# voidstar69/softray

Hardware: AMD Instinct MI355X
Metric: Mrays/s (primary rays) at 4096x4096, shading + 100-sample soft shadows, own BVH, frame read back to the host (higher is better)
Workload: dtype f64; 1 GPU; 1000000 random triangles (System.Random seed 12345, extent 0.05, unit cube) + BVH, 4096x4096, spp 1, shading + 100 shadow samples/hit, pose yaw135/pitch-22/depth 1.5; trace_mode=bvh, parallelism=one GPU

## Files before the change

softray_amd/csrc/sr_api.cpp:

```cpp
#include "../../include/softray.h"

#include <hip/hip_runtime.h>

#include <algorithm>
#include <climits>
#include <cmath>
#include <cstdio>
#include <cstdlib>
#include <cstring>
#include <memory>
#include <string>
#include <vector>

#include "sr_device.h"
#include "sr_host.h"
#include "sr_rccl.h"

namespace {

thread_local std::string g_err;

int fail(int code, const std::string& msg) {
    g_err = msg;
    return code;
// ... 8 lines not shown
        if (e__ != hipSuccess) return hip_fail(e__, #call);  \
    } while (0)

int rccl_fail(const sr::RcclApi* api, int rc, const char* what) {
    g_err = std::string(what) + ": " + (api && api->GetErrorString ? api->GetErrorString(rc) : "RCCL error") + " (" + std::to_string(rc) + ")";
    return SR_ERR_HIP;
}
#define SR_RCCL(api, call)                                        \
    do {                                                          \
        int r__ = (call);                                         \
        if (r__ != 0) return rccl_fail(api, r__, #call);          \
    } while (0)

struct DBuf {
    void*  p = nullptr;
    size_t cap = 0;
    hipError_t reserve(size_t bytes) {
        if (bytes <= cap && p) return hipSuccess;
        if (p) { hipError_t e = hipFree(p); p = nullptr; cap = 0; if (e != hipSuccess) return e; }
        size_t want = std::max<size_t>(bytes, 256);
        hipError_t e = hipMalloc(&p, want);
        if (e == hipSuccess) cap = want;
        return e;
    }
    template <class T> hipError_t upload(const std::vector<T>& v) {
        hipError_t e = reserve(v.size() * sizeof(T));
        if (e != hipSuccess || v.empty()) return e;
        return hipMemcpy(p, v.data(), v.size() * sizeof(T), hipMemcpyHostToDevice);
    }
    void release() { if (p) (void)hipFree(p); p = nullptr; cap = 0; }
};

}

struct sr_scene {
    int device = -1;
    std::vector<sr_scene*> parts;
    std::vector<double>   v9;
    std::vector<uint32_t> argb;
    double bmin[3] = {0, 0, 0}, bmax[3] = {0, 0, 0};
    double vmin[3] = {0, 0, 0}, vmax[3] = {0, 0, 0};
    bool have_model = false;
    size_t ntris = 0;
    const sr_scene* host_src = nullptr;
    bool host_model_stale = false;
    std::vector<sr::Rec128> tri_recs;
    std::vector<sr::Rec128> extra_recs;
    sr::RootBox root{};
    sr::RefTree ref;
    sr::Bvh     bvh;
    bool        bvh_on_device = false;
    size_t      bvh_num_nodes = 0;
    DBuf d_tris, d_extra, d_rnodes, d_rboxes, d_rleaf, d_bnodes, d_btris, d_bslab, d_v9, d_bcam;
    DBuf d_bounds;
    std::vector<int> b4_level_first;
    DBuf d_bdepth, d_tbox;
    bool bdepth_valid = false;
    double cam_origin[3] = {0, 0, 0};
    bool   cam_valid = false;
    DBuf   d_blight;
    bool   blight_valid = false;
    double blight_pos[3] = {0, 0, 0}, blight_radius = 0;
    DBuf   d_binter;
    bool   interior_valid = false;
    DBuf d_b4, d_b4cam, d_b4light;
    size_t b4_num = 0;
    int    b4_depth = 0;
    bool   b4cam_valid = false, b4light_valid = false;
    int    b4cam_known = 0, b4light_known = 0;
    DBuf   d_rng_cam, d_rng_light;
    bool   part_valid = false, part_cam = false, part_light = false;
    double part_origin[3] = {0, 0, 0}, part_lightpos[3] = {0, 0, 0}, part_radius = 0;
    double b4_light[3] = {0, 0, 0};
    double b4_light_radius = 0;
    uint32_t dbg_frame[3] = {0, 0, 0};
    hipEvent_t pre_ready = nullptr, pre_used = nullptr;
    bool pre_ready_set = false, pre_used_set = false;
    DBuf d_shadow_cache, d_static_claim, d_static_hits;
    DBuf d_ao_cache, d_ao_claim;
    DBuf d_aop_table, d_aop_rows, d_aop_state;
    DBuf d_pp_state;
    bool aop_rows_ready = false;
    std::unique_ptr<sr::NetRandom> aop_host_random;
    uint64_t aop_host_drawn = 0;
    bool ao_cache_empty = true;
    std::vector<uint8_t> ao_cache_host;
    std::vector<uint8_t> shadow_cache_host;
    int32_t ao_table_seed = 0;
    int  ao_table_rc = SR_OK;
    DBuf d_lf_cache, d_lf_claim, d_lf_points;
    int32_t lf_res = 64;
    bool lf_shadows = false;
    bool lf_interp = false;
    int32_t lf_points_res = 0;
    bool lf_cache_empty = true;
    std::vector<uint32_t> lf_cache_host;
    bool lf_tris = false;
    DBuf d_lft_cache, d_lft_claim, d_rhandle;
    bool lft_cache_empty = true;
    std::vector<uint32_t> lft_cache_host;
    DBuf d_pt_table;
    int32_t pt_table_seed = 0;
// ... 629 lines not shown
    const bool shadows_on_bvh = (fc.flags & SR_F_SHADOWS) && f->trace_mode == SR_MODE_REF_TREE && !(f->flags & SR_F_LITERAL_SECONDARY) && s->bvh.built && !static_shadows &&
                                (fc.flags & SR_F_POINT_LIGHT) && fc.shadow_samples <= kMaxShaftSamples && f->max_bounces == 0 &&
                                !(f->flags & (SR_F_SINGLE_KERNEL | SR_F_PER_LANE_SHADOWS)) && s->dbg[SR_DBG_LITERAL_SHADOWS] <= 0;
    if (shadows_on_bvh && (rc = sync_geometry(s, SR_MODE_BVH))) return rc;
    const bool bvh_walks = f->trace_mode == SR_MODE_BVH || shadows_on_bvh;
    const bool wide = bvh_walks && s->b4_num > 0 && s->dbg[SR_DBG_BVH2_PACKETS] <= 0;
    bool rewrote = false;
    const bool lf = (f->flags & SR_F_LIGHT_FIELD) != 0;
    const bool pkt_primary = f->trace_mode == SR_MODE_BVH && s->dbg[SR_DBG_PER_LANE_PRIMARY] <= 0 && !((f->flags & SR_F_FOCAL_BLUR) && f->sub_pixel_res > 1) && !lf && !pts;
    const bool want_cam = wide && pkt_primary, want_light = wide && (fc.flags & SR_F_SHADOWS) && (fc.flags & SR_F_POINT_LIGHT);
    if ((want_cam || want_light) && s->dbg[SR_DBG_KERNEL_SWITCH] != 71) {
        const auto same3 = [](const double* a, const double* b) { return a[0] == b[0] && a[1] == b[1] && a[2] == b[2]; };
        const bool cam_ok = !want_cam || (s->part_cam && same3(s->part_origin, fc.start_world));
        const bool light_ok = !want_light || (s->part_light && same3(s->part_lightpos, fc.light_pos_model) && s->part_radius == fc.light_radius);
        if (!s->part_valid || !cam_ok || !light_ok) {
            SR_HIP(s->d_rng_cam.reserve(s->b4_num * 4 * 8));
            SR_HIP(s->d_rng_light.reserve(s->b4_num * 4 * 8));
            rewrote = true;
            s->part_valid = false;
            s->cam_valid = false; s->b4cam_valid = false; s->b4light_valid = false;
            s->blight_valid = false;
            s->interior_valid = false;
            SR_HIP(sr::launch_facing_partition((const sr::Bvh4Node*)s->d_b4.p, (int)s->b4_num, (sr::Rec128*)s->d_btris.p, (sr::TriSlab*)s->d_bslab.p,
                                               fc.start_world, want_cam, fc.light_pos_model, fc.light_radius, want_light, s->d_rng_cam.p, s->d_rng_light.p, stream));
            s->part_cam = want_cam; s->part_light = want_light;
            for (int i = 0; i < 3; ++i) { s->part_origin[i] = fc.start_world[i]; s->part_lightpos[i] = fc.light_pos_model[i]; }
            s->part_radius = fc.light_radius;
            s->part_valid = true;
        }
    } else if (s->part_valid && s->dbg[SR_DBG_KERNEL_SWITCH] == 71) {
        s->part_valid = false; s->b4cam_valid = false; s->b4light_valid = false;
        s->blight_valid = false;
    }
    if (bvh_walks && (fc.flags & SR_F_SHADOWS) && (fc.flags & SR_F_POINT_LIGHT) && s->d_bslab.p && !s->interior_valid) {
        SR_HIP(s->d_binter.reserve(s->ntris));
        rewrote = true;
        SR_HIP(sr::launch_interior_flags(dev_scene(s), (int)s->ntris, (uint8_t*)s->d_binter.p, stream));
        s->interior_valid = true;
    }
    if (pkt_primary) {
        const size_t nt = s->ntris;
        const bool same_origin = s->cam_origin[0] == fc.start_world[0] && s->cam_origin[1] == fc.start_world[1] && s->cam_origin[2] == fc.start_world[2];
        if (!s->cam_valid || !same_origin) {
            SR_HIP(s->d_bcam.reserve(nt * sizeof(sr::CamCone)));
            rewrote = true;
            s->cam_valid = false;
            s->b4cam_valid = false;
            SR_HIP(sr::launch_cam_cones(dev_scene(s), (int)nt, fc.start_world, (sr::CamCone*)s->d_bcam.p, stream));
            for (int i = 0; i < 3; ++i) s->cam_origin[i] = fc.start_world[i];
            s->cam_valid = true;
        }
        if (wide && !s->b4cam_valid) {
            rewrote = true;
            int known, swap;
            point_outside_axes(s->root, fc.start_world, 0.0, known, swap);
            if (known != 7 || s->dbg[SR_DBG_KERNEL_SWITCH] == 61) known = swap = 0;
            SR_HIP(sr::launch_order_nodes((const sr::Bvh4Node*)s->d_b4.p, (sr::Bvh4Node*)s->d_b4cam.p, (int)s->b4_num, s->root, fc.start_world, false, swap,
                                          (s->part_valid && s->part_cam) ? s->d_rng_cam.p : nullptr, stream));
            s->b4cam_known = known;
            s->b4cam_valid = true;
        }
        if (wide) s->dbg_frame[0] |= (uint32_t)s->b4cam_known << 4;
    }
    if (wide && (fc.flags & SR_F_SHADOWS) && (fc.flags & SR_F_POINT_LIGHT)) {
        const bool same_light = s->b4_light[0] == fc.light_pos_model[0] && s->b4_light[1] == fc.light_pos_model[1] && s->b4_light[2] == fc.light_pos_model[2] &&
                                s->b4_light_radius == fc.light_radius;
        if (!s->b4light_valid || !same_light) {
            rewrote = true;
            s->b4light_valid = false;
            int known, beyond;
            point_outside_axes(s->root, fc.light_pos_model, fc.light_radius, known, beyond);
            if (s->dbg[SR_DBG_KERNEL_SWITCH] == 62) known = 0;
            SR_HIP(sr::launch_order_nodes((const sr::Bvh4Node*)s->d_b4.p, (sr::Bvh4Node*)s->d_b4light.p, (int)s->b4_num, s->root, fc.light_pos_model, true, known & ~beyond,
                                          (s->part_valid && s->part_light) ? s->d_rng_light.p : nullptr, stream));
            s->b4light_known = known;
            for (int i = 0; i < 3; ++i) s->b4_light[i] = fc.light_pos_model[i];
            s->b4_light_radius = fc.light_radius;
            s->b4light_valid = true;
        }
        s->dbg_frame[0] |= (uint32_t)s->b4light_known;
    }
    const bool shadows = (fc.flags & SR_F_SHADOWS) != 0;
    const bool shaft = shadows && bvh_walks && (fc.flags & SR_F_POINT_LIGHT) && !(f->flags & SR_F_PER_LANE_SHADOWS) &&
                       (fc.shadow_samples <= 128 || (fc.shadow_samples <= kMaxShaftSamples && !static_shadows));
    if (shaft && wide && s->b4light_valid && dev_scene(s).b4light && !(s->dbg[SR_DBG_PER_LANE_SHAFT] > 0 && (s->dbg[SR_DBG_PER_LANE_SHAFT] & 1)) &&
        s->dbg[SR_DBG_KERNEL_SWITCH] != 96) {
        const bool same_ball = s->blight_pos[0] == fc.light_pos_model[0] && s->blight_pos[1] == fc.light_pos_model[1] && s->blight_pos[2] == fc.light_pos_model[2] &&
                               s->blight_radius == fc.light_radius;
        if (!s->blight_valid || !same_ball) {
            s->blight_valid = false;
            if (s->d_blight.reserve(s->ntris * sizeof(sr::LightCone)) == hipSuccess) {
                rewrote = true;
                SR_HIP(sr::launch_light_cones(dev_scene(s), (int)s->ntris, fc.light_pos_model, fc.light_radius, (sr::LightCone*)s->d_blight.p, stream));
                for (int i = 0; i < 3; ++i) s->blight_pos[i] = fc.light_pos_model[i];
                s->blight_radius = fc.light_radius;
                s->blight_valid = true;
            } else {
                (void)hipGetLastError();
            }
        }
    } else if (s->dbg[SR_DBG_KERNEL_SWITCH] == 96) {
        s->blight_valid = false;
    }
    if (rewrote) {
        if (!s->pre_ready) SR_HIP(hipEventCreateWithFlags(&s->pre_ready, hipEventDisableTiming));
        SR_HIP(hipEventRecord(s->pre_ready, stream));
        s->pre_ready_set = true;
// ... 2603 lines not shown
```

softray_amd/csrc/sr_device.h:

```cpp
#pragma once
#include <hip/hip_runtime.h>
#include <stdint.h>

#include <vector>

#include "sr_types.h"

namespace sr {

struct DevScene {
    const Rec128*  tris;
    int32_t        ntris;
    const Rec128*  extra;
    int32_t        nextra;
    const RefNode* rnodes;
    const LeafBox* rboxes;
    const int32_t* rleaf;
    int32_t        rdepth;
    const BvhNode* bnodes;
    const Rec128*  btris;
    const TriSlab* bslab;
    const CamCone* bcam;
    const LightCone* blight;
    const double*  v9;
    int32_t        bdepth;
    int32_t        bnode_bits;
    const Bvh4Node* b4;
    const Bvh4Node* b4cam;
    const Bvh4Node* b4light;
    int32_t        b4depth;
    int32_t        b4cam_known, b4light_known;
    RootBox        root;
    uint8_t*       shadow_cache;
    const uint8_t* binter;
};

constexpr int kShaftRounds = 2;
enum KernelId { K_RENDER = 0, K_TRACE = 1, K_PRIMARY = 2, K_SHADOW = 3, K_RESOLVE = 4, K_SHAFT = 5, K_FALLBACK = 6, K_SHAFT2 = 7, K_SHADOW2 = 8, K_POST = 9, K_ANTI_ALIAS = 10, K_BOUNCE = 11, K_PATHTRACE = 12, K_PT_COUNT = 13, K_PT_EXCHANGE = 14, K_VOXEL_WALK = 15, K_VOXELISE = 16, K_AO = 17, K_AO_PROBE = 18, K_LF_LOOKUP = 19, K_LF_FILL = 20, K_LF_APPLY = 21, K_LF_BAKE = 22, K_TRI_RECORDS = 23, K_TRI_BOUNDS = 24, K_REFIT_LEAVES = 25, K_REFIT_NODES = 26, K_PTS_INGEST = 27, K_PTS_SORT = 28, K_LFI_LOOKUP = 29, K_LFI_APPLY = 30, K_LFT_FILL = 31, K_LFT_HIT = 32, K_LFT_TRACE = 33, K_LFT_BAKE = 34, K_HITS = 35, K_DRAWS = 36, K_AOP_PROBE = 37, K_PP_TRACE = 38, K_SSP_CLAIM = 39, K_SSP_APPLY = 40, K_COUNT = 41 };
const char* kernel_name(int id);

struct RenderLaunch {
    DevScene    sc;
    FrameConst  fc;
    int32_t     mode;
    const double* offsets;
    const int32_t* row_map;
    uint32_t*   pixels;
    unsigned long long* stats;
    hipStream_t stream;
};

hipError_t launch_render(const RenderLaunch& L);

struct HitsOut {
    double*   starts;
    double*   dirs;
    uint8_t*  hit;
    double*   ray_frac;
    double*   pos;
    double*   normal;
    uint32_t* color;
    int32_t*  tri;
};

struct PipelineLaunch {
    DevScene    sc;
    FrameConst  fc;
    int32_t     mode;
    const double*  offsets;
    const int32_t* row_map;
    uint32_t*   pixels;
// ... 165 lines not shown
    const double* pos;
    const double* nrm;
    const uint32_t* color;
    uint32_t*   out;
    uint32_t*   incoming;
    double*     dirs;
    uint64_t    first_sample;
    void*       rays;
    int32_t*    table;
    const NetState* windows;
    const uint32_t* stride_rows;
    int32_t*    base_window;
    uint32_t*   pass_units;
    hipError_t (*host_table)(void* user, uint64_t first_point, uint32_t count, int32_t* d_table, hipStream_t stream);
    unsigned int* counters;
    unsigned int* ray_sort_buf;
    void*       ray_sort_temp;
    size_t      ray_sort_temp_bytes;
    void*       bounce_prep;
    void*       bounce_res;
    int32_t*    bounce_stack;
    size_t      bounce_stack_bytes;
    bool        bvh2_packets;
    unsigned long long* stats;
    int32_t     persistent_blocks;
    hipStream_t stream;
    void (*get_events)(void* user, int kernel_id, hipEvent_t* start, hipEvent_t* stop);
    void*       user;
};
hipError_t launch_path_points(const PathPointsLaunch& L);
size_t path_points_table_bytes(int64_t pass);
hipError_t launch_order_nodes(const Bvh4Node* in, Bvh4Node* out, int num_nodes, const RootBox& root, const double point[3], bool far_first, int swap_mask,
                              const void* live_runs, hipStream_t stream);
hipError_t launch_facing_partition(const Bvh4Node* base, int num_nodes, Rec128* btris, TriSlab* bslab, const double origin[3], bool use_cam,
                                   const double light[3], double light_radius, bool use_light, void* cam_rng, void* light_rng, hipStream_t stream);
hipError_t launch_cam_cones(const DevScene& sc, int ntris, const double origin[3], CamCone* out, hipStream_t stream);
hipError_t launch_light_cones(const DevScene& sc, int ntris, const double light[3], double light_radius, LightCone* out, hipStream_t stream);
hipError_t launch_interior_flags(const DevScene& sc, int ntris, uint8_t* out, hipStream_t stream);
size_t pipeline_hit_record_bytes();
size_t pipeline_static_cells();
int pipeline_round_cap(int round);
int pipeline_round_cap_max(int round);
int pipeline_bounce_lds_levels();
int pipeline_pt_chunk();
size_t pipeline_round_state_bytes();
size_t pipeline_counter_bytes();
size_t pipeline_tile_items(int width, int rows, int n2);

hipError_t gather_records_device(int n, const unsigned int* d_order, const Rec128* d_tris, Rec128* d_btris, const TriSlab* d_slab_in,
                                 TriSlab* d_bslab, hipStream_t stream);
hipError_t build_bvh_device(const double* d_v9, int n, const RootBox& root, const Rec128* d_tris, const TriSlab* d_slab_in,
                            BvhNode* d_nodes, Rec128* d_btris, TriSlab* d_bslab, int* num_nodes, int* depth, hipStream_t stream, int leaf_max = 0);

size_t ray_sort_temp_bytes(unsigned int cap);
hipError_t ray_sort(const void* queue, const unsigned int* d_count, unsigned int cap, const RootBox& root, unsigned int* keys, unsigned int* keys2,
                    unsigned int* idx, unsigned int* order_out, void* temp, size_t temp_bytes, hipStream_t stream);

size_t point_order_temp_bytes(unsigned int cap);
unsigned int point_order_skip_mask(bool sorted);
hipError_t point_order(const void* recs, unsigned int n, bool sorted, const RootBox& root, unsigned int* keys, unsigned int* keys2, unsigned int* idx,
                       unsigned int* order_out, void* temp, size_t temp_bytes, hipStream_t stream);

hipError_t collapse_bvh4_device(const BvhNode* d_nodes, int num_nodes, Bvh4Node* d_wide, int* num_wide, int* depth, hipStream_t stream,
                                std::vector<int>* level_first = nullptr);

hipError_t make_slabs_device(const double* d_v9, int n, const RootBox& root, TriSlab* d_out, hipStream_t stream);
// ... 72 lines not shown
```

softray_amd/csrc/sr_kernels.hip:

```cpp
#include "sr_trace.h"

namespace sr {

extern __shared__ __attribute__((aligned(16))) unsigned char lds_raw[];

template <int MODE, bool EXTRA, bool LDSGEOM, bool STATS>
__global__ __launch_bounds__(256) void k_render(DevScene sc, FrameConst fc, const double* __restrict__ offsets,
                                                const int32_t* __restrict__ row_map, uint32_t* __restrict__ pixels,
                                                int stack_levels, unsigned long long* stats) {
    const int tid = threadIdx.x;
    const int wave = tid >> 6, lane = tid & 63;
    const int col = blockIdx.x * 16 + (wave & 1) * 8 + (lane & 7);
    const int crow = blockIdx.y * 16 + (wave >> 1) * 8 + (lane >> 3);

    int32_t* stack_mem = reinterpret_cast<int32_t*>(lds_raw);
    Stack st{stack_mem + tid, 256};
    const Rec128* tris = sc.tris;
    const Rec128* extra = sc.extra;
    if (LDSGEOM) {
        size_t off = ((size_t)stack_levels * 256 * 4 + 15) & ~(size_t)15;
        uint4* dst = reinterpret_cast<uint4*>(lds_raw + off);
        const int nt16 = (MODE != MODE_BVH ? sc.ntris : 0) * 8, ne16 = sc.nextra * 8;
        const uint4* srcT = reinterpret_cast<const uint4*>(sc.tris);
        const uint4* srcE = reinterpret_cast<const uint4*>(sc.extra);
// ... 89 lines not shown
        case K_PRIMARY: return "k_primary";
        case K_SHADOW: return "k_shadow";
        case K_RESOLVE: return "k_resolve";
        case K_SHAFT: return "k_shaft";
        case K_FALLBACK: return "k_shadow_fallback";
        case K_BOUNCE: return "k_bounce";
        case K_PATHTRACE: return "k_pathtrace";
        case K_PT_COUNT: return "k_pathtrace_count";
        case K_PT_EXCHANGE: return "pathtrace_exchange";
        case K_AO: return "ambient_occlusion";
        case K_AO_PROBE: return "k_ao_probe";
        case K_DRAWS: return "k_draws";
        case K_AOP_PROBE: return "k_aop_probe";
        case K_PP_TRACE: return "path_points_rays";
        case K_SSP_CLAIM: return "k_ssp_claim";
        case K_SSP_APPLY: return "k_ssp_apply";
        case K_LF_LOOKUP: return "k_lf_lookup";
        case K_LF_FILL: return "k_lf_fill";
        case K_LF_APPLY: return "k_lf_apply";
        case K_LFT_FILL: return "k_lft_fill";
        case K_LFT_HIT: return "k_lft_hit";
        case K_LFT_TRACE: return "k_lft_trace";
        case K_LFT_BAKE: return "k_lft_bake";
        case K_LF_BAKE: return "k_lf_bake";
        case K_LFI_LOOKUP: return "k_lfi_lookup";
        case K_LFI_APPLY: return "k_lfi_apply";
        case K_HITS: return "k_hits";
        case K_PTS_INGEST: return "k_pts_ingest";
        case K_PTS_SORT: return "k_pts_sort";
        case K_TRI_RECORDS: return "k_tri_records";
        case K_TRI_BOUNDS: return "k_tri_bounds";
        case K_REFIT_LEAVES: return "k_refit_leaves";
        case K_REFIT_NODES: return "k_refit_nodes";
        case K_VOXEL_WALK: return "k_voxel_walk";
        case K_VOXELISE: return "voxelise";
        case K_SHAFT2: return "k_shaft_round2";
        case K_SHADOW2: return "k_shadow_round2";
        case K_POST: return "k_post_process";
        case K_ANTI_ALIAS: return "k_anti_alias";
        default: return "?";
    }
}

static int stack_levels_for(const DevScene& sc, int mode) {
    if (mode == MODE_REF) return sc.rdepth + 2;
    if (mode == MODE_BVH) return sc.bdepth + 2;
    return 1;
}

static const size_t kLdsGeomBudget = 96 * 1024;

template <int MODE, bool EXTRA, bool LDSGEOM>
static hipError_t launch_render_t(const RenderLaunch& L, dim3 grid, size_t lds, int levels) {
    if (L.stats)
        hipLaunchKernelGGL((k_render<MODE, EXTRA, LDSGEOM, true>), grid, dim3(256), lds, L.stream, L.sc, L.fc, L.offsets,
                           L.row_map, L.pixels, levels, L.stats);
    else
        hipLaunchKernelGGL((k_render<MODE, EXTRA, LDSGEOM, false>), grid, dim3(256), lds, L.stream, L.sc, L.fc, L.offsets,
                           L.row_map, L.pixels, levels, L.stats);
    return hipGetLastError();
}

template <int MODE>
static hipError_t launch_render_m(const RenderLaunch& L) {
    dim3 grid((L.fc.width + 15) / 16, (L.fc.num_rows + 15) / 16);
    if (grid.x == 0 || grid.y == 0) return hipSuccess;
// ... 59 lines not shown
```

softray_amd/csrc/sr_lbvh.hip:

```cpp
#include "sr_device.h"

#include <hipcub/hipcub.hpp>

#include <algorithm>
#include <vector>

namespace sr {

namespace {

constexpr int kLeafMaxDefault = 4;

struct FBox { float lo[3], hi[3]; };

__device__ __forceinline__ unsigned long long spread21(unsigned long long x) {
    x &= 0x1fffffull;
    x = (x | x << 32) & 0x1f00000000ffffull;
    x = (x | x << 16) & 0x1f0000ff0000ffull;
    x = (x | x << 8) & 0x100f00f00f00f00full;
    x = (x | x << 4) & 0x10c30c30c30c30c3ull;
    x = (x | x << 2) & 0x1249249249249249ull;
    return x;
}

__device__ __forceinline__ FBox tri_box(const double lo[3], const double hi[3], const double centre[3], float pad) {
    FBox b;
    for (int a = 0; a < 3; ++a) {
        b.lo[a] = __double2float_rd(lo[a] - centre[a] - (double)pad);
        b.hi[a] = __double2float_ru(hi[a] - centre[a] + (double)pad);
    }
    return b;
}

// ... 304 lines not shown
            b = empty_box();
            if (ch->n0 >= 0) b = merge(b, load_box(ch->lo0, ch->hi0));
            if (ch->n1 >= 0) b = merge(b, load_box(ch->lo1, ch->hi1));
        }
        if (side == 0) store_box(nd->lo0, nd->hi0, b); else store_box(nd->lo1, nd->hi1, b);
    }
}

__global__ void __launch_bounds__(256) k_refit_nodes2(int num_nodes, BvhNode* nodes, const FBox* __restrict__ tbox, const uint8_t* __restrict__ depth,
                                                      int level) {
    const int i = blockIdx.x * blockDim.x + threadIdx.x;
    if (i >= num_nodes || depth[i] != level) return;
    refit_node2(nodes, i, tbox);
}

__global__ void __launch_bounds__(256) k_refit_nodes4(int first, int count, Bvh4Node* wide, int num_wide, const FBox* __restrict__ tbox) {
    const int t = blockIdx.x * blockDim.x + threadIdx.x;
    if (t >= count) return;
    Bvh4Node* nd = wide + first + t;
    for (int j = 0; j < 4; ++j) {
        const int c = nd->ch[j].c, cn = nd->ch[j].n;
        if (cn < 0) continue;
        FBox b;
        if (cn > 0) b = leaf_box(tbox, c, cn);
        else {
            if (c <= first + t || c >= num_wide) continue;
            const Bvh4Node* ch = wide + c;
            b = empty_box();
            for (int k = 0; k < 4; ++k)
                if (ch->ch[k].n >= 0) b = merge(b, load_box(ch->ch[k].lo, ch->ch[k].hi));
        }
        store_box(nd->ch[j].lo, nd->ch[j].hi, b);
    }
}

__global__ void k_collapse_level(const BvhNode* __restrict__ nodes, const int2* __restrict__ in, int n_in, int2* __restrict__ out,
                                 int* __restrict__ counters , Bvh4Node* __restrict__ wide) {
    const int i = blockIdx.x * blockDim.x + threadIdx.x;
    if (i >= n_in) return;
    const int2 item = in[i];
    Bvh4Child ch[4];
    int k = 0;
    const auto child_of = [](const BvhNode& n, int side) {
        Bvh4Child c;
        for (int a = 0; a < 3; ++a) { c.lo[a] = side ? n.lo1[a] : n.lo0[a]; c.hi[a] = side ? n.hi1[a] : n.hi0[a]; }
        c.c = side ? n.c1 : n.c0;
        c.n = side ? n.n1 : n.n0;
        return c;
    };
    const auto area = [](const Bvh4Child& c) {
        const float dx = c.hi[0] - c.lo[0], dy = c.hi[1] - c.lo[1], dz = c.hi[2] - c.lo[2];
        return dx * dy + dy * dz + dz * dx;
    };
    {
        const BvhNode r = nodes[item.x];
        const Bvh4Child a = child_of(r, 0), b = child_of(r, 1);
        if (a.n >= 0) ch[k++] = a;
        if (b.n >= 0) ch[k++] = b;
    }
    while (k < 4) {
        int best = -1;
        float best_area = -1.0f;
        for (int j = 0; j < k; ++j)
            if (ch[j].n == 0) { const float a = area(ch[j]); if (a > best_area) { best_area = a; best = j; } }
        if (best < 0) break;
        const BvhNode m = nodes[ch[best].c];
// ... 192 lines not shown
```

softray_amd/csrc/sr_pipeline.hip:

```cpp
#include "sr_trace.h"
#include "sr_light_cone.h"
#include "sr_umbra_hint.h"

#include <algorithm>
#include <type_traits>

namespace sr {

extern __shared__ __attribute__((aligned(16))) unsigned char lds_pipe[];

struct alignas(16) HitRec {
    double   pos[3];
    double   nrm[3];
    uint32_t sample;
    uint32_t pad[3];
};
static_assert(sizeof(HitRec) == 64, "HitRec must be 64 bytes");
constexpr uint32_t kInvalidHit = 0xffffffffu;

__device__ __forceinline__ void finish_hit(const DevScene& sc, const FrameConst& fc, uint32_t* samples, uint32_t sample, uint32_t cell,
                                           uint32_t shaded, double frac) {
    if (fc.flags & 32u) {
        uint32_t v = (uint32_t)(int)(frac * 254 + 1) & 0xffu;
        sc.shadow_cache[cell] = (uint8_t)(v ? v : 1u);
// ... 4527 lines not shown
        const double* p = btris[k].p;
        const double mag = 1e-9 * (1.0 + fabs(p[3]) + fabs(ox) + fabs(oy) + fabs(oz) + fabs(lx) + fabs(ly) + fabs(lz));
        const bool cam_dead = use_cam && (p[0] * ox + p[1] * oy + p[2] * oz - p[3]) < -mag;
        const bool light_dead = use_light && (p[0] * lx + p[1] * ly + p[2] * lz - p[3]) + R * 1.000001 < -mag;
        return cam_dead ? (light_dead ? 3 : 0) : (light_dead ? 2 : 1);
    };
    int pos = c, cnt[4] = {0, 0, 0, 0};
#pragma unroll
    for (int g = 0; g < 3; ++g) {
        for (int k = pos; k < c + n; ++k) {
            if (group(k) != g) continue;
            if (k != pos) {
                uint4* a = reinterpret_cast<uint4*>(&btris[k]); uint4* b = reinterpret_cast<uint4*>(&btris[pos]);
                for (int w = 0; w < 8; ++w) { const uint4 x = a[w]; a[w] = b[w]; b[w] = x; }
                uint4* sa_ = reinterpret_cast<uint4*>(&bslab[k]); uint4* sb_ = reinterpret_cast<uint4*>(&bslab[pos]);
                for (int w = 0; w < 4; ++w) { const uint4 x = sa_[w]; sa_[w] = sb_[w]; sb_[w] = x; }
            }
            ++pos;
            if (g == 0) cnt[0]++; else if (g == 1) cnt[1]++; else cnt[2]++;
        }
    }
    cam_rng[t] = make_int2(cnt[0], cnt[1] + cnt[2]);
    light_rng[t] = make_int2(0, cnt[0] + cnt[1]);
}

hipError_t launch_facing_partition(const Bvh4Node* base, int num_nodes, Rec128* btris, TriSlab* bslab, const double origin[3], bool use_cam,
                                   const double light[3], double light_radius, bool use_light, void* cam_rng, void* light_rng, hipStream_t stream) {
    if (num_nodes <= 0) return hipSuccess;
    hipLaunchKernelGGL(k_facing_partition, dim3((unsigned)((num_nodes * 4 + 255) / 256)), dim3(256), 0, stream, base, num_nodes, btris, bslab,
                       origin[0], origin[1], origin[2], use_cam ? 1 : 0, light[0], light[1], light[2], light_radius, use_light ? 1 : 0, (int2*)cam_rng, (int2*)light_rng);
    return hipGetLastError();
}

__global__ __launch_bounds__(256) void k_order_nodes(const Bvh4Node* __restrict__ in, Bvh4Node* __restrict__ out, int n, float px, float py, float pz, int far_first,
                                                     int swap_mask, const int2* __restrict__ rng) {
    const int i = blockIdx.x * 256 + threadIdx.x;
    if (i >= n) return;
    Bvh4Node nd = in[i];
    if (rng) {
#pragma unroll
        for (int k = 0; k < 4; ++k) {
            if (nd.ch[k].n > 0) {
                const int2 r = rng[i * 4 + k];
                nd.ch[k].c += r.x;
                nd.ch[k].n = r.y > 0 ? r.y : -1;
            }
        }
    }
    float key[4];
#pragma unroll
    for (int k = 0; k < 4; ++k) {
        const Bvh4Child& c = nd.ch[k];
        const float cx = 0.5f * (c.lo[0] + c.hi[0]) - px, cy = 0.5f * (c.lo[1] + c.hi[1]) - py, cz = 0.5f * (c.lo[2] + c.hi[2]) - pz;
        const float d2 = cx * cx + cy * cy + cz * cz;
        key[k] = c.n < 0 ? FLT_MAX : (far_first ? -d2 : d2);
    }
#pragma unroll
    for (int a = 1; a < 4; ++a) {
#pragma unroll
        for (int b = a; b > 0; --b) {
            if (key[b] < key[b - 1]) {
                const float tk = key[b]; key[b] = key[b - 1]; key[b - 1] = tk;
                const Bvh4Child tc = nd.ch[b]; nd.ch[b] = nd.ch[b - 1]; nd.ch[b - 1] = tc;
            }
        }
    }
#pragma unroll
    for (int k = 0; k < 4; ++k)
#pragma unroll
        for (int a = 0; a < 3; ++a)
            if ((swap_mask >> a) & 1) { const float t = nd.ch[k].lo[a]; nd.ch[k].lo[a] = nd.ch[k].hi[a]; nd.ch[k].hi[a] = t; }
    if (far_first) {
#pragma unroll
        for (int k = 0; k < 4; ++k) {
            const float lz = nd.ch[k].lo[2], hx = nd.ch[k].hi[0], hy = nd.ch[k].hi[1];
            nd.ch[k].lo[2] = hx; nd.ch[k].hi[0] = hy; nd.ch[k].hi[1] = lz;
        }
    }
    out[i] = nd;
}

hipError_t launch_order_nodes(const Bvh4Node* in, Bvh4Node* out, int num_nodes, const RootBox& root, const double point[3], bool far_first, int swap_mask,
                              const void* live_runs, hipStream_t stream) {
    if (num_nodes <= 0) return hipSuccess;
    hipLaunchKernelGGL(k_order_nodes, dim3((unsigned)((num_nodes + 255) / 256)), dim3(256), 0, stream, in, out, num_nodes,
                       (float)(point[0] - root.centre[0]), (float)(point[1] - root.centre[1]), (float)(point[2] - root.centre[2]), far_first ? 1 : 0, swap_mask,
                       (const int2*)live_runs);
    return hipGetLastError();
}

hipError_t launch_cam_cones(const DevScene& sc, int ntris, const double origin[3], CamCone* out, hipStream_t stream) {
    if (ntris <= 0) return hipSuccess;
    hipLaunchKernelGGL(k_cam_cones, dim3((unsigned)((ntris + 255) / 256)), dim3(256), 0, stream, sc.btris, sc.bslab, sc.v9, ntris,
                       origin[0], origin[1], origin[2], out);
    return hipGetLastError();
}

static int pipe_stack_levels(const DevScene& sc, int mode) {
    if (mode == MODE_REF) return sc.rdepth + 2;
    if (mode == MODE_BVH) return sc.bdepth + 2;
    return 1;
}

constexpr int kHeadsPrimary = 64, kHeadsShaft = kHeadsPrimary + 8 * kTileHeadStride, kCounterWords = kHeadsShaft + 8 * kTileHeadStride;
static unsigned tile_grid(const PipelineLaunch& L, unsigned virtual_blocks, int wgs_per_cu, unsigned int* heads, unsigned int** heads_out) {
    const unsigned resident = (unsigned)(L.persistent_blocks / 8 * wgs_per_cu);
    const bool persistent = virtual_blocks > resident && L.fc.debug != 81 && (virtual_blocks & 7u) == 0u;
    *heads_out = persistent ? heads : nullptr;
    return persistent ? resident : virtual_blocks;
}

template <int MODE, bool EXTRA, bool SUB, int PKT>
static hipError_t launch_primary_p(const PipelineLaunch& L, int row_begin, int row_count, uint32_t* samples, int pad_tiles) {
    const unsigned vblocks = (unsigned)xcd_tile_grid(L.fc.width, row_count);
    unsigned int* heads;
    dim3 grid(tile_grid(L, vblocks, SUB ? 5 : 6, L.counters + kHeadsPrimary, &heads));
    if (heads && L.fc.debug != 82) { heads = nullptr; grid = dim3(vblocks); }
// ... 1160 lines not shown
```

Baseline: 2640 Mrays/s.

## Refit wide BVH boxes tightly around facing-partitioned live triangle runs

When camera- or light-facing partitions have shrunk each leaf to a live triangle run, rebuild the wide-BVH child boxes bottom-up so they bound only the live triangles, then reorder the nodes in place. Tighter boxes are meant to cut node visits and triangle tests for primary and shadow rays. It adds per-level refit kernel launches and a single-block top pass whenever the camera or light copy is rebuilt, and debug switches can restrict how many levels are tightened.

```diff
diff --git a/softray_amd/csrc/sr_api.cpp b/softray_amd/csrc/sr_api.cpp
--- a/softray_amd/csrc/sr_api.cpp
+++ b/softray_amd/csrc/sr_api.cpp
@@ -64,6 +64,8 @@
 };
 
 }
+
+constexpr int kTightNone = -2, kTightCut = -1;
 
 struct sr_scene {
     int device = -1;
@@ -100,6 +102,7 @@
     int    b4_depth = 0;
     bool   b4cam_valid = false, b4light_valid = false;
     int    b4cam_known = 0, b4light_known = 0;
+    int    b4cam_tight = kTightNone, b4light_tight = kTightNone;
     DBuf   d_rng_cam, d_rng_light;
     bool   part_valid = false, part_cam = false, part_light = false;
     double part_origin[3] = {0, 0, 0}, part_lightpos[3] = {0, 0, 0}, part_radius = 0;
@@ -795,6 +798,21 @@
         s->part_valid = false; s->b4cam_valid = false; s->b4light_valid = false;
         s->blight_valid = false;
     }
+    const auto tight_wanted = [&](const void* runs, bool light_copy) {
+        const int64_t sw = s->dbg[SR_DBG_KERNEL_SWITCH];
+        if (!runs || sw == 72 || sw == (light_copy ? 73 : 74) || s->b4_level_first.size() < 2 || s->b4_level_first.back() != (int)s->b4_num || !s->d_v9.p) return kTightNone;
+        return sw >= 75 && sw <= 79 ? (int)(sw - 74) : kTightCut;
+    };
+    const auto tighten = [&](void* copy, const void* runs, int cut) -> int {
+        int rc2;
+        hipEvent_t e0, e1;
+        if ((rc2 = next_events(s, sr::K_TIGHT_BOXES, e0, e1))) return rc2;
+        if (e0) SR_HIP(hipEventRecord(e0, stream));
+        SR_HIP(sr::tight_boxes_device((const sr::Bvh4Node*)s->d_b4.p, (sr::Bvh4Node*)copy, (int)s->b4_num, s->b4_level_first, runs, (const sr::Rec128*)s->d_btris.p,
+                                      (const double*)s->d_v9.p, (int)s->ntris, s->root, cut, stream));
+        if (e1) SR_HIP(hipEventRecord(e1, stream));
+        return SR_OK;
+    };
     if (bvh_walks && (fc.flags & SR_F_SHADOWS) && (fc.flags & SR_F_POINT_LIGHT) && s->d_bslab.p && !s->interior_valid) {
         SR_HIP(s->d_binter.reserve(s->ntris));
         rewrote = true;
@@ -813,13 +831,21 @@
             for (int i = 0; i < 3; ++i) s->cam_origin[i] = fc.start_world[i];
             s->cam_valid = true;
         }
+        if (wide && s->b4cam_valid && s->b4cam_tight != tight_wanted((s->part_valid && s->part_cam) ? s->d_rng_cam.p : nullptr, false)) s->b4cam_valid = false;
         if (wide && !s->b4cam_valid) {
             rewrote = true;
             int known, swap;
             point_outside_axes(s->root, fc.start_world, 0.0, known, swap);
             if (known != 7 || s->dbg[SR_DBG_KERNEL_SWITCH] == 61) known = swap = 0;
-            SR_HIP(sr::launch_order_nodes((const sr::Bvh4Node*)s->d_b4.p, (sr::Bvh4Node*)s->d_b4cam.p, (int)s->b4_num, s->root, fc.start_world, false, swap,
-                                          (s->part_valid && s->part_cam) ? s->d_rng_cam.p : nullptr, stream));
+            const void* runs = (s->part_valid && s->part_cam) ? s->d_rng_cam.p : nullptr;
+            const int cut = tight_wanted(runs, false);
+            if (cut != kTightNone) {
+                if ((rc = tighten(s->d_b4cam.p, runs, cut))) return rc;
+                SR_HIP(sr::launch_order_nodes((const sr::Bvh4Node*)s->d_b4cam.p, (sr::Bvh4Node*)s->d_b4cam.p, (int)s->b4_num, s->root, fc.start_world, false, swap, nullptr, stream));
+            } else {
+                SR_HIP(sr::launch_order_nodes((const sr::Bvh4Node*)s->d_b4.p, (sr::Bvh4Node*)s->d_b4cam.p, (int)s->b4_num, s->root, fc.start_world, false, swap, runs, stream));
+            }
+            s->b4cam_tight = cut;
             s->b4cam_known = known;
             s->b4cam_valid = true;
         }
@@ -828,14 +854,23 @@
     if (wide && (fc.flags & SR_F_SHADOWS) && (fc.flags & SR_F_POINT_LIGHT)) {
         const bool same_light = s->b4_light[0] == fc.light_pos_model[0] && s->b4_light[1] == fc.light_pos_model[1] && s->b4_light[2] == fc.light_pos_model[2] &&
                                 s->b4_light_radius == fc.light_radius;
-        if (!s->b4light_valid || !same_light) {
+        const void* lruns = (s->part_valid && s->part_light) ? s->d_rng_light.p : nullptr;
+        if (!s->b4light_valid || !same_light || s->b4light_tight != tight_wanted(lruns, true)) {
             rewrote = true;
             s->b4light_valid = false;
             int known, beyond;
             point_outside_axes(s->root, fc.light_pos_model, fc.light_radius, known, beyond);
             if (s->dbg[SR_DBG_KERNEL_SWITCH] == 62) known = 0;
-            SR_HIP(sr::launch_order_nodes((const sr::Bvh4Node*)s->d_b4.p, (sr::Bvh4Node*)s->d_b4light.p, (int)s->b4_num, s->root, fc.light_pos_model, true, known & ~beyond,
-                                          (s->part_valid && s->part_light) ? s->d_rng_light.p : nullptr, stream));
+            const int cut = tight_wanted(lruns, true);
+            if (cut != kTightNone) {
+                if ((rc = tighten(s->d_b4light.p, lruns, cut))) return rc;
+                SR_HIP(sr::launch_order_nodes((const sr::Bvh4Node*)s->d_b4light.p, (sr::Bvh4Node*)s->d_b4light.p, (int)s->b4_num, s->root, fc.light_pos_model, true,
+                                              known & ~beyond, nullptr, stream));
+            } else {
+                SR_HIP(sr::launch_order_nodes((const sr::Bvh4Node*)s->d_b4.p, (sr::Bvh4Node*)s->d_b4light.p, (int)s->b4_num, s->root, fc.light_pos_model, true, known & ~beyond,
+                                              lruns, stream));
+            }
+            s->b4light_tight = cut;
             s->b4light_known = known;
             for (int i = 0; i < 3; ++i) s->b4_light[i] = fc.light_pos_model[i];
             s->b4_light_radius = fc.light_radius;
diff --git a/softray_amd/csrc/sr_device.h b/softray_amd/csrc/sr_device.h
--- a/softray_amd/csrc/sr_device.h
+++ b/softray_amd/csrc/sr_device.h
@@ -36,7 +36,7 @@
 };
 
 constexpr int kShaftRounds = 2;
-enum KernelId { K_RENDER = 0, K_TRACE = 1, K_PRIMARY = 2, K_SHADOW = 3, K_RESOLVE = 4, K_SHAFT = 5, K_FALLBACK = 6, K_SHAFT2 = 7, K_SHADOW2 = 8, K_POST = 9, K_ANTI_ALIAS = 10, K_BOUNCE = 11, K_PATHTRACE = 12, K_PT_COUNT = 13, K_PT_EXCHANGE = 14, K_VOXEL_WALK = 15, K_VOXELISE = 16, K_AO = 17, K_AO_PROBE = 18, K_LF_LOOKUP = 19, K_LF_FILL = 20, K_LF_APPLY = 21, K_LF_BAKE = 22, K_TRI_RECORDS = 23, K_TRI_BOUNDS = 24, K_REFIT_LEAVES = 25, K_REFIT_NODES = 26, K_PTS_INGEST = 27, K_PTS_SORT = 28, K_LFI_LOOKUP = 29, K_LFI_APPLY = 30, K_LFT_FILL = 31, K_LFT_HIT = 32, K_LFT_TRACE = 33, K_LFT_BAKE = 34, K_HITS = 35, K_DRAWS = 36, K_AOP_PROBE = 37, K_PP_TRACE = 38, K_SSP_CLAIM = 39, K_SSP_APPLY = 40, K_COUNT = 41 };
+enum KernelId { K_RENDER = 0, K_TRACE = 1, K_PRIMARY = 2, K_SHADOW = 3, K_RESOLVE = 4, K_SHAFT = 5, K_FALLBACK = 6, K_SHAFT2 = 7, K_SHADOW2 = 8, K_POST = 9, K_ANTI_ALIAS = 10, K_BOUNCE = 11, K_PATHTRACE = 12, K_PT_COUNT = 13, K_PT_EXCHANGE = 14, K_VOXEL_WALK = 15, K_VOXELISE = 16, K_AO = 17, K_AO_PROBE = 18, K_LF_LOOKUP = 19, K_LF_FILL = 20, K_LF_APPLY = 21, K_LF_BAKE = 22, K_TRI_RECORDS = 23, K_TRI_BOUNDS = 24, K_REFIT_LEAVES = 25, K_REFIT_NODES = 26, K_PTS_INGEST = 27, K_PTS_SORT = 28, K_LFI_LOOKUP = 29, K_LFI_APPLY = 30, K_LFT_FILL = 31, K_LFT_HIT = 32, K_LFT_TRACE = 33, K_LFT_BAKE = 34, K_HITS = 35, K_DRAWS = 36, K_AOP_PROBE = 37, K_PP_TRACE = 38, K_SSP_CLAIM = 39, K_SSP_APPLY = 40, K_TIGHT_BOXES = 41, K_COUNT = 42 };
 const char* kernel_name(int id);
 
 struct RenderLaunch {
@@ -268,6 +268,8 @@
 size_t path_points_table_bytes(int64_t pass);
 hipError_t launch_order_nodes(const Bvh4Node* in, Bvh4Node* out, int num_nodes, const RootBox& root, const double point[3], bool far_first, int swap_mask,
                               const void* live_runs, hipStream_t stream);
+hipError_t tight_boxes_device(const Bvh4Node* d_base, Bvh4Node* d_out, int num_wide, const std::vector<int>& level_first, const void* d_live_runs,
+                              const Rec128* d_btris, const double* d_v9, int ntris, const RootBox& root, int cut, hipStream_t stream);
 hipError_t launch_facing_partition(const Bvh4Node* base, int num_nodes, Rec128* btris, TriSlab* bslab, const double origin[3], bool use_cam,
                                    const double light[3], double light_radius, bool use_light, void* cam_rng, void* light_rng, hipStream_t stream);
 hipError_t launch_cam_cones(const DevScene& sc, int ntris, const double origin[3], CamCone* out, hipStream_t stream);
diff --git a/softray_amd/csrc/sr_kernels.hip b/softray_amd/csrc/sr_kernels.hip
--- a/softray_amd/csrc/sr_kernels.hip
+++ b/softray_amd/csrc/sr_kernels.hip
@@ -145,6 +145,7 @@
         case K_TRI_BOUNDS: return "k_tri_bounds";
         case K_REFIT_LEAVES: return "k_refit_leaves";
         case K_REFIT_NODES: return "k_refit_nodes";
+        case K_TIGHT_BOXES: return "k_tight_boxes";
         case K_VOXEL_WALK: return "k_voxel_walk";
         case K_VOXELISE: return "voxelise";
         case K_SHAFT2: return "k_shaft_round2";
diff --git a/softray_amd/csrc/sr_lbvh.hip b/softray_amd/csrc/sr_lbvh.hip
--- a/softray_amd/csrc/sr_lbvh.hip
+++ b/softray_amd/csrc/sr_lbvh.hip
@@ -1,4 +1,5 @@
 #include "sr_device.h"
+#include "sr_tight_boxes.h"
 
 #include <hipcub/hipcub.hpp>
 
@@ -369,6 +370,97 @@
         }
         store_box(nd->ch[j].lo, nd->ch[j].hi, b);
     }
+}
+
+struct TightArgs {
+    const Bvh4Node* base;
+    Bvh4Node*       out;
+    int             num_wide;
+    const int2*     rng;
+    const Rec128*   btris;
+    const double*   v9;
+    int             ntris;
+    double          centre[3];
+    float           pad;
+};
+__device__ __forceinline__ void tight_slot(const TightArgs& A, int node, int slot, bool tighten) {
+    Bvh4Child ch = A.base[node].ch[slot];
+    if (ch.n > 0) {
+        const int2 r = A.rng[node * 4 + slot];
+        bool ok = tighten && ch.c >= 0 && ch.n <= A.ntris - ch.c;
+        if (ok && r.x >= 0 && r.y <= ch.n - r.x)
+            for (int k = 0; k < r.y; ++k) { const int tri = A.btris[ch.c + r.x + k].aux; ok = ok && tri >= 0 && tri < A.ntris; }
+        tight_leaf_slot(ch, r.x, r.y, ok, [&](int k) {
+            const double* p = A.v9 + (size_t)A.btris[k].aux * 9;
+            double lo[3], hi[3];
+            for (int a = 0; a < 3; ++a) {
+                lo[a] = fmin(fmin(p[a], p[3 + a]), p[6 + a]);
+                hi[a] = fmax(fmax(p[a], p[3 + a]), p[6 + a]);
+            }
+            const FBox b = tri_box(lo, hi, A.centre, A.pad);
+            TightBox t;
+            for (int a = 0; a < 3; ++a) { t.lo[a] = b.lo[a]; t.hi[a] = b.hi[a]; }
+            return t;
+        });
+    } else if (ch.n == 0 && tighten && ch.c > node && ch.c < A.num_wide) {
+        const Bvh4Node below = A.out[ch.c];
+        tight_inner_slot(ch, below);
+    }
+    A.out[node].ch[slot] = ch;
+}
+__global__ void __launch_bounds__(256) k_tight_level(TightArgs A, int first, int count, int tighten) {
+    const int t = blockIdx.x * blockDim.x + threadIdx.x;
+    if (t >= count * 4) return;
+    tight_slot(A, first + (t >> 2), t & 3, tighten != 0);
+}
+constexpr int kTightTopLevels = 16, kTightTopNodes = 4096, kTightTopThreads = 1024;
+struct TightTop { int levels; int first_tight; int first[kTightTopLevels + 1]; };
+__global__ void __launch_bounds__(kTightTopThreads) k_tight_top(TightArgs A, TightTop top) {
+    for (int lv = top.levels - 1; lv >= 0; --lv) {
+        const int first = top.first[lv], slots = (top.first[lv + 1] - first) * 4;
+        for (int t = threadIdx.x; t < slots; t += kTightTopThreads) tight_slot(A, first + (t >> 2), t & 3, lv >= top.first_tight);
+        __syncthreads();
+    }
+}
+
+hipError_t tight_boxes_device(const Bvh4Node* d_base, Bvh4Node* d_out, int num_wide, const std::vector<int>& level_first, const void* d_live_runs,
+                              const Rec128* d_btris, const double* d_v9, int ntris, const RootBox& root, int cut, hipStream_t stream) {
+    if (num_wide <= 0 || ntris <= 0 || !d_live_runs) return hipErrorInvalidValue;
+    if (level_first.size() < 2 || level_first.front() != 0 || level_first.back() != num_wide) return hipErrorInvalidValue;
+    for (size_t lv = 0; lv + 1 < level_first.size(); ++lv)
+        if (level_first[lv] > level_first[lv + 1]) return hipErrorInvalidValue;
+    double ext = 0;
+    for (int a = 0; a < 3; ++a) ext = std::max(ext, root.max[a] - root.min[a]);
+    TightArgs A;
+    A.base = d_base; A.out = d_out; A.num_wide = num_wide; A.rng = (const int2*)d_live_runs; A.btris = d_btris; A.v9 = d_v9; A.ntris = ntris;
+    for (int a = 0; a < 3; ++a) A.centre[a] = root.centre[a];
+    A.pad = (float)std::ldexp(ext > 0 ? ext : 1.0, -16);
+    const int levels = (int)level_first.size() - 1;
+    const int first_tight = tight_first_level(levels, cut);
+    int top = 0;
+    while (top < levels && top < kTightTopLevels && level_first[top + 1] <= kTightTopNodes) ++top;
+    const int T = 256;
+    for (int lv = levels - 1; lv >= std::max(top, first_tight); --lv) {
+        const int first = level_first[lv], count = level_first[lv + 1] - first;
+        if (count <= 0) continue;
+        hipLaunchKernelGGL(k_tight_level, dim3((unsigned)(((size_t)count * 4 + T - 1) / T)), dim3(T), 0, stream, A, first, count, 1);
+        LB_HIP(hipGetLastError());
+    }
+    if (first_tight > top) {
+        const int first = level_first[top], count = level_first[first_tight] - first;
+        if (count > 0) {
+            hipLaunchKernelGGL(k_tight_level, dim3((unsigned)(((size_t)count * 4 + T - 1) / T)), dim3(T), 0, stream, A, first, count, 0);
+            LB_HIP(hipGetLastError());
+        }
+    }
+    if (top > 0) {
+        TightTop tt;
+        tt.levels = top; tt.first_tight = first_tight;
+        for (int lv = 0; lv <= kTightTopLevels; ++lv) tt.first[lv] = level_first[std::min(lv, top)];
+        hipLaunchKernelGGL(k_tight_top, dim3(1), dim3(kTightTopThreads), 0, stream, A, tt);
+        LB_HIP(hipGetLastError());
+    }
+    return hipSuccess;
 }
 
 __global__ void k_collapse_level(const BvhNode* __restrict__ nodes, const int2* __restrict__ in, int n_in, int2* __restrict__ out,
diff --git a/softray_amd/csrc/sr_pipeline.hip b/softray_amd/csrc/sr_pipeline.hip
--- a/softray_amd/csrc/sr_pipeline.hip
+++ b/softray_amd/csrc/sr_pipeline.hip
@@ -4583,6 +4583,39 @@
     return hipGetLastError();
 }
 
+__device__ __forceinline__ void order_node(Bvh4Node& nd, float px, float py, float pz, int far_first, int swap_mask) {
+    float key[4];
+#pragma unroll
+    for (int k = 0; k < 4; ++k) {
+        const Bvh4Child& c = nd.ch[k];
+        const float cx = 0.5f * (c.lo[0] + c.hi[0]) - px, cy = 0.5f * (c.lo[1] + c.hi[1]) - py, cz = 0.5f * (c.lo[2] + c.hi[2]) - pz;
+        const float d2 = cx * cx + cy * cy + cz * cz;
+        key[k] = c.n < 0 ? FLT_MAX : (far_first ? -d2 : d2);
+    }
+#pragma unroll
+    for (int a = 1; a < 4; ++a) {
+#pragma unroll
+        for (int b = a; b > 0; --b) {
+            if (key[b] < key[b - 1]) {
+                const float tk = key[b]; key[b] = key[b - 1]; key[b - 1] = tk;
+                const Bvh4Child tc = nd.ch[b]; nd.ch[b] = nd.ch[b - 1]; nd.ch[b - 1] = tc;
+            }
+        }
+    }
+#pragma unroll
+    for (int k = 0; k < 4; ++k)
+#pragma unroll
+        for (int a = 0; a < 3; ++a)
+            if ((swap_mask >> a) & 1) { const float t = nd.ch[k].lo[a]; nd.ch[k].lo[a] = nd.ch[k].hi[a]; nd.ch[k].hi[a] = t; }
+    if (far_first) {
+#pragma unroll
+        for (int k = 0; k < 4; ++k) {
+            const float lz = nd.ch[k].lo[2], hx = nd.ch[k].hi[0], hy = nd.ch[k].hi[1];
+            nd.ch[k].lo[2] = hx; nd.ch[k].hi[0] = hy; nd.ch[k].hi[1] = lz;
+        }
+    }
+}
+
 __global__ __launch_bounds__(256) void k_order_nodes(const Bvh4Node* __restrict__ in, Bvh4Node* __restrict__ out, int n, float px, float py, float pz, int far_first,
                                                      int swap_mask, const int2* __restrict__ rng) {
     const int i = blockIdx.x * 256 + threadIdx.x;
@@ -4598,42 +4631,26 @@
             }
         }
     }
-    float key[4];
-#pragma unroll
-    for (int k = 0; k < 4; ++k) {
-        const Bvh4Child& c = nd.ch[k];
-        const float cx = 0.5f * (c.lo[0] + c.hi[0]) - px, cy = 0.5f * (c.lo[1] + c.hi[1]) - py, cz = 0.5f * (c.lo[2] + c.hi[2]) - pz;
-        const float d2 = cx * cx + cy * cy + cz * cz;
-        key[k] = c.n < 0 ? FLT_MAX : (far_first ? -d2 : d2);
-    }
-#pragma unroll
-    for (int a = 1; a < 4; ++a) {
-#pragma unroll
-        for (int b = a; b > 0; --b) {
-            if (key[b] < key[b - 1]) {
-                const float tk = key[b]; key[b] = key[b - 1]; key[b - 1] = tk;
-                const Bvh4Child tc = nd.ch[b]; nd.ch[b] = nd.ch[b - 1]; nd.ch[b - 1] = tc;
-            }
-        }
-    }
-#pragma unroll
-    for (int k = 0; k < 4; ++k)
-#pragma unroll
-        for (int a = 0; a < 3; ++a)
-            if ((swap_mask >> a) & 1) { const float t = nd.ch[k].lo[a]; nd.ch[k].lo[a] = nd.ch[k].hi[a]; nd.ch[k].hi[a] = t; }
-    if (far_first) {
-#pragma unroll
-        for (int k = 0; k < 4; ++k) {
-            const float lz = nd.ch[k].lo[2], hx = nd.ch[k].hi[0], hy = nd.ch[k].hi[1];
-            nd.ch[k].lo[2] = hx; nd.ch[k].hi[0] = hy; nd.ch[k].hi[1] = lz;
-        }
-    }
+    order_node(nd, px, py, pz, far_first, swap_mask);
     out[i] = nd;
+}
+__global__ __launch_bounds__(256) void k_order_nodes_inplace(Bvh4Node* nodes, int n, float px, float py, float pz, int far_first, int swap_mask) {
+    const int i = blockIdx.x * 256 + threadIdx.x;
+    if (i >= n) return;
+    Bvh4Node nd = nodes[i];
+    order_node(nd, px, py, pz, far_first, swap_mask);
+    nodes[i] = nd;
 }
 
 hipError_t launch_order_nodes(const Bvh4Node* in, Bvh4Node* out, int num_nodes, const RootBox& root, const double point[3], bool far_first, int swap_mask,
                               const void* live_runs, hipStream_t stream) {
     if (num_nodes <= 0) return hipSuccess;
+    if (in == out) {
+        if (live_runs) return hipErrorInvalidValue;
+        hipLaunchKernelGGL(k_order_nodes_inplace, dim3((unsigned)((num_nodes + 255) / 256)), dim3(256), 0, stream, out, num_nodes,
+                           (float)(point[0] - root.centre[0]), (float)(point[1] - root.centre[1]), (float)(point[2] - root.centre[2]), far_first ? 1 : 0, swap_mask);
+        return hipGetLastError();
+    }
     hipLaunchKernelGGL(k_order_nodes, dim3((unsigned)((num_nodes + 255) / 256)), dim3(256), 0, stream, in, out, num_nodes,
                        (float)(point[0] - root.centre[0]), (float)(point[1] - root.centre[1]), (float)(point[2] - root.centre[2]), far_first ? 1 : 0, swap_mask,
                        (const int2*)live_runs);
diff --git a/softray_amd/csrc/sr_tight_boxes.h b/softray_amd/csrc/sr_tight_boxes.h
--- /dev/null
+++ b/softray_amd/csrc/sr_tight_boxes.h
@@ -0,0 +1,52 @@
+#pragma once
+#include <math.h>
+#include <stdint.h>
+
+#include "sr_types.h"
+
+namespace sr {
+
+struct TightBox { float lo[3], hi[3]; };
+
+SR_HOST_DEVICE inline TightBox tight_empty() {
+    TightBox b;
+    for (int a = 0; a < 3; ++a) { b.lo[a] = INFINITY; b.hi[a] = -INFINITY; }
+    return b;
+}
+SR_HOST_DEVICE inline TightBox tight_union(const TightBox& x, const TightBox& y) {
+    TightBox b;
+    for (int a = 0; a < 3; ++a) { b.lo[a] = fminf(x.lo[a], y.lo[a]); b.hi[a] = fmaxf(x.hi[a], y.hi[a]); }
+    return b;
+}
+
+SR_HOST_DEVICE inline int tight_first_level(int num_levels, int cut) {
+    return (cut < 0 || cut >= num_levels) ? 0 : num_levels - cut;
+}
+
+template <class BoxOf>
+SR_HOST_DEVICE inline void tight_leaf_slot(Bvh4Child& ch, int run_first, int run_count, bool tighten, BoxOf box_of) {
+    if (run_first < 0 || run_count > ch.n - run_first) return;
+    if (run_count <= 0) { ch.c += run_first; ch.n = -1; return; }
+    ch.c += run_first;
+    ch.n = run_count;
+    if (!tighten) return;
+    TightBox b = box_of(ch.c);
+    for (int k = 1; k < run_count; ++k) b = tight_union(b, box_of(ch.c + k));
+    for (int a = 0; a < 3; ++a) { ch.lo[a] = b.lo[a]; ch.hi[a] = b.hi[a]; }
+}
+
+SR_HOST_DEVICE inline void tight_inner_slot(Bvh4Child& ch, const Bvh4Node& below) {
+    TightBox b = tight_empty();
+    bool any = false;
+    for (int k = 0; k < 4; ++k) {
+        if (below.ch[k].n < 0) continue;
+        TightBox c;
+        for (int a = 0; a < 3; ++a) { c.lo[a] = below.ch[k].lo[a]; c.hi[a] = below.ch[k].hi[a]; }
+        b = tight_union(b, c);
+        any = true;
+    }
+    if (!any) { ch.n = -1; return; }
+    for (int a = 0; a < 3; ++a) { ch.lo[a] = b.lo[a]; ch.hi[a] = b.hi[a]; }
+}
+
+}
```

Result: faster. 2899 Mrays/s (median of 6 runs) (+9.8%).
